# HKUST-Aerial-Robotics/FIESTA

Hardware: NVIDIA H100
Metric: esdf_voxel_updates_per_s (higher is better)
Workload: dtype int32+f64

## Files before the change

### fiesta_b200/csrc/fb_exact.cu

```cuda
#include <cub/cub.cuh>
#include <stdio.h>
#include <stdlib.h>
#include <algorithm>
#include <chrono>
#include "fb_common.cuh"
#include "fb_exact.h"

#define XNONE 0xffffffffu
#define XMB_NONE 0xffffffffffffffffull

__device__ __forceinline__ void x_coords(const FbGeom &g, uint32_t ii, int &x, int &y, int &z) {
  z = ii % (unsigned)g.pz; const unsigned xy = ii / (unsigned)g.pz; y = xy % (unsigned)g.gy; x = xy / (unsigned)g.gy;
}
__device__ __forceinline__ unsigned x_d2(int x, int y, int z, uint32_t c) {
  int ox, oy, oz; fb_unpack(c, ox, oy, oz); ox -= x; oy -= y; oz -= z;
  return (unsigned)(ox * ox + oy * oy + oz * oz);
}
__device__ __forceinline__ unsigned x_dist_of(int x, int y, int z, uint32_t c) { return c < 2u ? 0xffffffffu : x_d2(x, y, z, c); }

__global__ void k_x_flag_exist(const uint32_t *list, unsigned n, const double *occ, double l_occ, uint8_t *flags, int want) {
  const unsigned i = blockIdx.x * blockDim.x + threadIdx.x;
  if (i < n) flags[i] = ((occ[list[i]] > l_occ) ? 1 : 0) == want;
}
__global__ void k_x_apply_seed(FbGeom g, const uint32_t *E, unsigned n, uint32_t *cobs, unsigned long long *LS, unsigned long long t0) {
// ... 17 lines not shown
  const unsigned i = blockIdx.x * blockDim.x + threadIdx.x;
  if (i < n) scratch[sel[i]] = i;
}
__global__ void k_x_scan_deps(FbGeom g, const uint32_t *cobs, const uint32_t *occbits, const uint32_t *rank, const unsigned long long *LS,
                              unsigned long long *k1, unsigned long long *k2, uint32_t *dv, unsigned *ndep, unsigned cap, int shift) {
  for (long long v = (long long)blockIdx.x * blockDim.x + threadIdx.x; v < g.ptotal; v += (long long)gridDim.x * blockDim.x) {
    const uint32_t c = cobs[v] & FB_CODE_MASK;
    bool dep = false;
    unsigned r = 0;
    if (c >= 2u) {
      int ox, oy, oz; fb_unpack(c, ox, oy, oz);
      const long long oi = fb_ii(g, ox, oy, oz);
      if (!((__ldg(&occbits[oi >> 5]) >> (oi & 31)) & 1u)) { r = rank[oi]; dep = r != XNONE; }
    }
    const unsigned slot = fb_warp_append(ndep, dep);
    if (dep && slot < cap) {
      const unsigned long long inv = ~LS[v];
      if (shift) k1[slot] = ((unsigned long long)r << shift) | (inv & ((1ull << shift) - 1ull));
      else { k1[slot] = r; k2[slot] = inv; }
      dv[slot] = (uint32_t)v;
    }
  }
}
__global__ void k_x_unset(const uint32_t *list, unsigned n, uint32_t *scratch) {
  const unsigned i = blockIdx.x * blockDim.x + threadIdx.x;
  if (i < n) scratch[list[i]] = XNONE;
}
__global__ void k_x_iota(uint32_t *a, unsigned n) { const unsigned i = blockIdx.x * blockDim.x + threadIdx.x; if (i < n) a[i] = i; }
__global__ void k_x_gather64(const unsigned long long *src, const uint32_t *idx, unsigned n, unsigned long long *dst) {
  const unsigned i = blockIdx.x * blockDim.x + threadIdx.x; if (i < n) dst[i] = src[idx[i]];
}
__global__ void k_x_gather32(const uint32_t *src, const uint32_t *idx, unsigned n, uint32_t *dst) {
  const unsigned i = blockIdx.x * blockDim.x + threadIdx.x; if (i < n) dst[i] = src[idx[i]];
}
__global__ void k_x_set_ord(const uint32_t *deps, unsigned n, uint32_t *ord) {
  const unsigned i = blockIdx.x * blockDim.x + threadIdx.x;
  if (i < n) ord[deps[i]] = i;
}
__global__ void k_x_fill32(uint32_t *a, size_t n, uint32_t val) {
  for (size_t i = (size_t)blockIdx.x * blockDim.x + threadIdx.x; i < n; i += (size_t)gridDim.x * blockDim.x) a[i] = val;
}
__global__ void k_x_fill64(unsigned long long *a, size_t n, unsigned long long val) {
  for (size_t i = (size_t)blockIdx.x * blockDim.x + threadIdx.x; i < n; i += (size_t)gridDim.x * blockDim.x) a[i] = val;
}

static inline unsigned nblk(size_t n, unsigned t = 256) { return (unsigned)((n + t - 1) / t); }

static int x_select(FbExact *X, const uint32_t *in, const uint8_t *flags, uint32_t *out, unsigned n, unsigned *count, cudaStream_t s) {
  *count = 0;
  if (n == 0) return FIESTA_OK;
  size_t bytes = 0;
  CK(cub::DeviceSelect::Flagged(nullptr, bytes, in, flags, out, X->d_count.p, (int)n, s));
  CK(X->cub_tmp.grow(bytes, s));
  CK(cub::DeviceSelect::Flagged(X->cub_tmp.p, bytes, in, flags, out, X->d_count.p, (int)n, s));
  CK(cudaMemcpyAsync(X->h_count, X->d_count, 4, cudaMemcpyDeviceToHost, s));
  CK(cudaStreamSynchronize(s));
  *count = *X->h_count;
  return FIESTA_OK;
}
static int x_sort_pairs(FbExact *X, const unsigned long long *kin, unsigned long long *kout, const uint32_t *vin, uint32_t *vout, unsigned n, cudaStream_t s,
                        int key_bits = 64) {
  size_t bytes = 0;
  CK(cub::DeviceRadixSort::SortPairs(nullptr, bytes, kin, kout, vin, vout, (int)n, 0, key_bits, s));
  CK(X->cub_tmp.grow(bytes, s));
  CK(cub::DeviceRadixSort::SortPairs(X->cub_tmp.p, bytes, kin, kout, vin, vout, (int)n, 0, key_bits, s));
  return FIESTA_OK;
}
int fb_exact_init(FbExact *X, const FbGeom &g, int device, cudaStream_t s) {
  const size_t P = (size_t)g.ptotal;
  CK(fb_xrelax_init());
  X->relax_blocks = fb_xrelax_blocks(device);
  if (X->relax_blocks <= 0 || X->relax_blocks > FB_X_MAX_BLOCKS) { fb_set_error("exact mode init: k_x_relax does not fit on this device"); return FIESTA_ERR_CUDA; }
  CK(X->MB.alloc(P)); CK(X->LS.alloc(P)); CK(X->tkey.alloc(P));
  CK(X->touched.alloc(P));
  CK(X->SUM.alloc(P)); CK(X->SUMg.alloc(P)); CK(cudaMemsetAsync(X->SUMg, 0, P * 4, s));
  CK(X->emask.alloc(P));
  CK(X->wstamp.alloc(P)); CK(cudaMemsetAsync(X->wstamp, 0, P * 4, s));
  for (int k = 0; k < 3; ++k) { CK(X->W[k].alloc(P)); CK(X->F[k].alloc(P)); CK(cudaMemsetAsync(X->W[k], 0, P * 4, s)); }
  for (int k = 0; k < 2; ++k) CK(X->E[k].alloc(P));
  X->dense_min = 16384u;
  if (const char *e = getenv("FIESTA_X_DENSE")) { long v = atol(e); if (v >= 0 && v <= (1 << 24)) X->dense_min = (unsigned)v; }
  if (const char *e = getenv("FIESTA_X_ASYNC")) X->async = atol(e) != 0;
  if (const char *e = getenv("FIESTA_X_SMALL_ASYNC")) X->small_async = atol(e) != 0;
  X->small_max = FB_X_SMALL_DEFAULT;
  if (const char *e = getenv("FIESTA_X_SMALL")) { long v = atol(e); if (v >= 0 && v <= 65536) X->small_max = (unsigned)v; }
  CK(X->slotc.alloc(((size_t)X->small_max + 1) * 32));
  const size_t c0 = P / 8 > (1u << 20) ? P / 8 : (1u << 20);
  for (FbDevBuf<unsigned long long> *b : {&X->k1, &X->k2, &X->k1b, &X->k2b}) CK(b->grow(c0, s));
  for (FbDevBuf<uint32_t> *b : {&X->dv, &X->idx[0], &X->idx[1], &X->deps, &X->nc[0], &X->nc[1], &X->sel}) CK(b->grow(c0, s));
  CK(X->flags.grow(c0, s));
  CK(X->cub_tmp.grow(c0 * 16 + (64u << 20), s));
  CK(X->d_ctl.alloc(1)); CK(cudaMemsetAsync(X->d_ctl, 0, sizeof(FbXCtl), s));
  CK(X->h_ctl.alloc(1));
  CK(X->d_count.alloc(4)); CK(X->d_flag.alloc(4));
  CK(X->h_count.alloc(4));
  CK(cudaMemsetAsync(X->d_count, 0, 16, s)); CK(cudaMemsetAsync(X->d_flag, 0, 16, s));
  k_x_fill64<<<FB_SMS * 8, 256, 0, s>>>(X->MB, P, XMB_NONE);
  CK(cudaMemsetAsync(X->tkey, 0, P * 8, s));
  CK(cudaMemsetAsync(X->LS, 0, P * 8, s));
  X->tclock = 1; X->key_base = 0; X->key_epoch = 1; X->key_hi = 1ull << FB_KEY_BITS; X->gen_id = 0; X->wclock = 0; X->sclock = 0;
  CK(cudaGetLastError());
  return FIESTA_OK;
}

int fb_exact_queue_crossings(FbExact *X, const unsigned long long *ins_key, const uint32_t *ins_vox, const unsigned long long *del_key,
                             const uint32_t *del_vox, FbDevBuf<uint32_t> &ins, unsigned *n_ins, FbDevBuf<uint32_t> &del, unsigned *n_del,
                             cudaStream_t s, int *launches) {
  int r;
  CK(cudaMemcpyAsync(X->h_count, X->d_count, 8, cudaMemcpyDeviceToHost, s));
  CK(cudaStreamSynchronize(s));
  const unsigned ni = X->h_count[0], nd = X->h_count[1];
  CK(ins.grow((size_t)*n_ins + ni, s, *n_ins));
  CK(del.grow((size_t)*n_del + nd, s, *n_del));
  CK(X->k1b.grow(ni > nd ? ni : nd, s));
  if (ni) { if ((r = x_sort_pairs(X, ins_key, X->k1b, ins_vox, ins + *n_ins, ni, s, FB_KEY_BITS))) return r; *n_ins += ni; *launches += 1; }
  if (nd) { if ((r = x_sort_pairs(X, del_key, X->k1b, del_vox, del + *n_del, nd, s, FB_KEY_BITS))) return r; *n_del += nd; *launches += 1; }
  return FIESTA_OK;
}
int fb_exact_next_epoch(FbExact *X, const FbGeom &g, cudaStream_t s) {
  X->key_base = 0;
  if (++X->key_epoch >= (1u << (64 - FB_KEY_BITS))) {
    CK(cudaMemsetAsync(X->tkey, 0, (size_t)g.ptotal * 8, s));
    X->key_epoch = 1;
  }
  X->key_hi = (unsigned long long)X->key_epoch << FB_KEY_BITS;
  return FIESTA_OK;
}

int fb_exact_update_esdf(FbExact *X, const FbGeom &g, uint32_t *cobs, uint32_t *scratch, const double *occ, const uint32_t *occbits, double l_occ,
                         const uint32_t *ins, unsigned n_ins, const uint32_t *del, unsigned n_del, cudaStream_t s, FbExactStats *st, int *launches) {
  int r;
  const size_t P = (size_t)g.ptotal;
  memset(st, 0, sizeof(*st));
  CK(X->flags.grow((size_t)(n_ins > n_del ? n_ins : n_del) + 16, s));
  static const bool xdbg = getenv("FIESTA_DEBUG_X") != nullptr;
  auto now = [] { return std::chrono::steady_clock::now(); };
  auto ms = [](std::chrono::steady_clock::time_point a, std::chrono::steady_clock::time_point b) { return std::chrono::duration<double, std::milli>(b - a).count(); };
  const auto t_begin = now();
  unsigned nE = 0, ndep_run = 0;
  unsigned long long ls_deps = 0;
  bool scratch_ok = X->scratch_clean;
  if (n_ins) {
    k_x_flag_exist<<<nblk(n_ins), 256, 0, s>>>(ins, n_ins, occ, l_occ, X->flags, 1);
    if ((r = x_select(X, ins, X->flags, X->E[0], n_ins, &nE, s))) return r;
    if (nE) k_x_apply_seed<<<nblk(nE), 256, 0, s>>>(g, X->E[0], nE, cobs, X->LS, X->tclock);
    X->tclock += nE;
    *launches += 2;
  }
  if (n_del) {
    CK(X->sel.grow((size_t)n_del + 16, s));
    if (!X->scratch_clean) { k_x_fill32<<<FB_SMS * 8, 256, 0, s>>>(scratch, P, XNONE); *launches += 1; }
    scratch_ok = true;
    X->scratch_clean = false;
    k_x_del_minpos<<<nblk(n_del), 256, 0, s>>>(del, n_del, occ, l_occ, scratch);
    k_x_del_flag<<<nblk(n_del), 256, 0, s>>>(del, n_del, occ, l_occ, scratch, X->flags);
    unsigned nd = 0;
    if ((r = x_select(X, del, X->flags, X->sel, n_del, &nd, s))) return r;
    k_x_unset<<<nblk(n_del), 256, 0, s>>>(del, n_del, scratch);
    *launches += 3;
    if (nd) {
      k_x_del_rank<<<nblk(nd), 256, 0, s>>>(X->sel, nd, scratch);
      int rank_bits = 1; while ((1ull << rank_bits) < (unsigned long long)nd) ++rank_bits;
      int clock_bits = 1; while (clock_bits < 64 && (X->tclock >> clock_bits)) ++clock_bits;
      const bool two_sorts = getenv("FIESTA_X_TWO_SORTS") != nullptr;
      const int shift = (rank_bits + clock_bits <= 64 && !two_sorts) ? 64 - rank_bits : 0;
      unsigned ndep = 0;
      for (int attempt = 0; attempt < 2; ++attempt) {
        const size_t cap = std::min({X->dv.cap, X->k1.cap, X->k2.cap});
        CK(cudaMemsetAsync(X->d_count, 0, 4, s));
        k_x_scan_deps<<<FB_SMS * 16, 256, 0, s>>>(g, cobs, occbits, scratch, X->LS, X->k1, X->k2, X->dv, X->d_count, (unsigned)cap, shift);
        CK(cudaMemcpyAsync(X->h_count, X->d_count, 4, cudaMemcpyDeviceToHost, s));
        CK(cudaStreamSynchronize(s));
        ndep = *X->h_count;
        *launches += 1;
        if (ndep <= cap) break;
        CK(X->dv.grow(ndep, s));
        CK(X->k1.grow(ndep, s));
        CK(X->k2.grow(ndep, s));
      }
      st->dependants = ndep;
      k_x_unset<<<nblk(nd), 256, 0, s>>>(X->sel, nd, scratch);
      if (ndep) {
        CK(X->k1b.grow(ndep, s));
        CK(X->k2b.grow(ndep, s));
        CK(X->idx[0].grow(ndep, s));
        CK(X->idx[1].grow(ndep, s));
        CK(X->deps.grow(ndep, s));
        CK(X->nc[0].grow(ndep, s));
        CK(X->nc[1].grow(ndep, s));
        CK(X->flags.grow(ndep, s));
        if (shift) {
          if ((r = x_sort_pairs(X, X->k1, X->k1b, X->dv, X->deps, ndep, s))) return r;
          *launches += 1;
        } else {
          k_x_iota<<<nblk(ndep), 256, 0, s>>>(X->idx[0], ndep);
          if ((r = x_sort_pairs(X, X->k2, X->k2b, X->idx[0], X->idx[1], ndep, s))) return r;
          k_x_gather64<<<nblk(ndep), 256, 0, s>>>(X->k1, X->idx[1], ndep, X->k1b);
          if ((r = x_sort_pairs(X, X->k1b, X->k2b, X->idx[1], X->idx[0], ndep, s))) return r;
          k_x_gather32<<<nblk(ndep), 256, 0, s>>>(X->dv, X->idx[0], ndep, X->deps);
          *launches += 5;
        }
        k_x_set_ord<<<nblk(ndep), 256, 0, s>>>(X->deps, ndep, scratch);
        *launches += 1;
        ndep_run = ndep; ls_deps = X->tclock;
        X->tclock += ndep;
      }
    }
  }
  st->generations = 0;
  if (xdbg) { cudaStreamSynchronize(s); fprintf(stderr, "[x] seeds+deletes %.2f ms (dependants %u)\n", ms(t_begin, now()), st->dependants); }
  if (nE || ndep_run) {
    if (xdbg && !X->d_dbg) CK(X->d_dbg.alloc(FB_X_DBG_WORDS));
    if (xdbg) CK(cudaMemsetAsync(X->d_dbg, 0, FB_X_DBG_WORDS * 8, s));
    if (X->sclock > 0xf0000000u) { CK(cudaMemsetAsync(X->SUMg, 0, P * 4, s)); X->sclock = 0; }
    if (X->gen_id > 0xf0000000u) X->gen_id = 0;
    if (X->wclock > 0xf0000000u) { CK(cudaMemsetAsync(X->wstamp, 0, P * 4, s)); X->wclock = 0; }
    FbXCtl *h = X->h_ctl;
    memset(h, 0, sizeof(*h));
    h->gen_id = X->gen_id; h->wclock = X->wclock; h->tclock = X->tclock; h->sclock = X->sclock; h->nE0 = nE;
    CK(cudaMemcpyAsync(X->d_ctl, h, sizeof(FbXCtl), cudaMemcpyHostToDevice, s));
    CK(fb_xrelax_launch(X, g, cobs, X->deps, ndep_run, scratch, X->nc[0], X->nc[1], occbits, ls_deps, xdbg ? X->d_dbg.p : nullptr, s));
    if (ndep_run) k_x_unset<<<nblk(ndep_run), 256, 0, s>>>(X->deps, ndep_run, scratch);
    CK(cudaMemcpyAsync(h, X->d_ctl, sizeof(FbXCtl), cudaMemcpyDeviceToHost, s));
    CK(cudaStreamSynchronize(s));
    *launches += ndep_run ? 2 : 1;
    if (h->err) {
      if (h->err == 3u) {
        for (int k = 0; k < 3; ++k) CK(cudaMemsetAsync(X->W[k], 0, P * 4, s));
        CK(cudaMemsetAsync(X->wstamp, 0, P * 4, s));
        X->wclock = 0;
      }
      fb_set_error(h->err == 1u ? "exact mode: generation with more than 2^27 entries"
                   : h->err == 3u ? "exact mode: a wait of the asynchronous work queue exceeded its bound" : "exact mode: behaviour fixpoint did not converge");
      return FIESTA_ERR_CUDA;
    }
    X->gen_id = h->gen_id; X->wclock = h->wclock; X->tclock = h->tclock; X->sclock = h->sclock;
    st->generations = h->generations; st->reseed_rounds = h->reseed_rounds; st->eval_rounds = h->rounds; st->dense_rounds = h->dense_rounds;
    st->voxels_changed = h->voxels_changed; st->expansions = h->expansions;
    if (xdbg) {
      static unsigned long long hd[FB_X_DBG_WORDS];
      static double cyc_per_us = 0;
      if (cyc_per_us == 0) { int dev = 0, khz = 0; CK(cudaGetDevice(&dev)); CK(cudaDeviceGetAttribute(&khz, cudaDevAttrClockRate, dev)); cyc_per_us = khz / 1000.0; }
      CK(cudaMemcpy(hd, X->d_dbg, sizeof(hd), cudaMemcpyDeviceToHost));
      static const char *cat[FB_XDBG_NCAT] = {"S", "round1", "rounds", "dense", "commit", "apply", "s.round1", "s.rounds", "s.commit", "s.apply", "top",
                                              "empty-barrier", "reseed.classify", "reseed.assemble", "", "", "async", "", "refresh", "s.async",
                                              "reseed.closure", "reseed.choose", "reseed.resolve", ""};
      fprintf(stderr, "[x] reseed rounds %u; phases (us, count):", st->reseed_rounds);
      for (int c = 0; c < FB_XDBG_NCAT; ++c)
        if (*cat[c]) fprintf(stderr, " %s %.0f/%llu", cat[c], hd[FB_XDBG_PHASE + 2 * c] / cyc_per_us, hd[FB_XDBG_PHASE + 2 * c + 1]);
      fprintf(stderr, "\n");
      fprintf(stderr, "[x] round work (summed longest CTA work time us / summed list length):");
      for (int c : {1, 2, 3, 6, 7}) fprintf(stderr, " %s %.0f/%llu", cat[c], hd[FB_XDBG_WORK + 2 * c] / cyc_per_us, hd[FB_XDBG_WORK + 2 * c + 1]);
      fprintf(stderr, "\n");
      for (int h = 0; h < 2; ++h) {
        fprintf(stderr, "[x] list-length histogram %s (log2 bucket=rounds):", h ? "s.rounds" : "rounds");
        for (int b = 0; b < 32; ++b) if (hd[FB_XDBG_NWH + 32 * h + b]) fprintf(stderr, " %d=%llu", b, hd[FB_XDBG_NWH + 32 * h + b]);
        fprintf(stderr, "\n");
      }
      fprintf(stderr, "[x] async: evaluations %llu dirty %llu pushes %llu spin %.0f us\n", hd[FB_XDBG_Q + 0], hd[FB_XDBG_Q + 1], hd[FB_XDBG_Q + 2],
              hd[FB_XDBG_Q + 3] / cyc_per_us);
      for (int gq = 0; gq < 2; ++gq) { fprintf(stderr, "[x] gen %d work lists:", gq); for (int r = 0; r < 512 && hd[FB_XDBG_ROUNDS + gq * 512 + r]; ++r) fprintf(stderr, " %llu", hd[FB_XDBG_ROUNDS + gq * 512 + r]); fprintf(stderr, "\n"); }
      fprintf(stderr, "[x] work-list entries: evaluated %llu refreshed %llu\n", hd[FB_XDBG_PHASE + 2 * 14], hd[FB_XDBG_PHASE + 2 * 14 + 1]);
      fprintf(stderr, "[x] reseed: dependants %u final after classify %llu closure rounds %llu list entries %llu resolve passes %llu\n", st->dependants,
              hd[FB_XDBG_PHASE + 2 * 15], hd[FB_XDBG_PHASE + 2 * 20 + 1], hd[FB_XDBG_PHASE + 2 * 15 + 1], hd[FB_XDBG_PHASE + 2 * 22 + 1]);
      fprintf(stderr, "[x] gens %u rounds %u dense %u deps %u nE0 %u |", st->generations, st->eval_rounds, st->dense_rounds, st->dependants, nE);
      for (unsigned q = 0; q < st->generations && q < FB_XDBG_GENS; ++q) fprintf(stderr, " %llu/%llu/%.1fus", hd[3 * q], hd[3 * q + 1], hd[3 * q + 2] / cyc_per_us);
      fprintf(stderr, "\n");
    }
  }
  X->scratch_clean = scratch_ok;
  return FIESTA_OK;
}
```

### fiesta_b200/csrc/fb_exact.h

```cpp
#pragma once
#include "fb_common.cuh"

#define FB_X_MAX_BLOCKS 256
#define FB_X_SMALL_DEFAULT 32768u
#define FB_XDBG_GENS 1024
#define FB_XDBG_NCAT 24
#define FB_XDBG_NQ 8
#define FB_XDBG_PHASE (3 * FB_XDBG_GENS)
#define FB_XDBG_ROUNDS (FB_XDBG_PHASE + 2 * FB_XDBG_NCAT)
#define FB_XDBG_WMAX (FB_XDBG_ROUNDS + 2 * 512)
#define FB_XDBG_WORK (FB_XDBG_WMAX + 4096)
#define FB_XDBG_NWH (FB_XDBG_WORK + 2 * FB_XDBG_NCAT)
#define FB_XDBG_Q (FB_XDBG_NWH + 2 * 32)
#define FB_X_DBG_WORDS (FB_XDBG_Q + FB_XDBG_NQ)

struct FbExactStats {
  unsigned long long expansions;
  unsigned long long voxels_changed;
  unsigned generations, eval_rounds, dense_rounds, dependants;
  unsigned reseed_rounds;
};

struct FbXCtl {
  unsigned bar, err;
  unsigned sclock;
  unsigned rbar;
  unsigned nE0;
  unsigned nW[3], nF[3];
  unsigned gen_id, wclock;
  unsigned generations, rounds, dense_rounds, reseed_rounds;
  unsigned long long tclock, expansions, voxels_changed;
  unsigned partial[FB_X_MAX_BLOCKS];
  alignas(128) unsigned long long qtail;
  alignas(128) unsigned qhead;
  alignas(128) unsigned qdone;
};

struct FbExact {
  FbDevBuf<unsigned long long> MB;
  FbDevBuf<unsigned long long> LS;
  FbDevBuf<unsigned long long> tkey;
  FbDevBuf<uint32_t> touched;
  unsigned long long tclock = 0;
  unsigned long long key_base = 0;
  unsigned long long key_hi = 0;
  unsigned key_epoch = 0;
  FbDevBuf<unsigned> d_count, d_flag;
  FbHostBuf<unsigned> h_count;
  bool scratch_clean = false;
  FbDevBuf<uint4> SUM;
  FbDevBuf<uint32_t> SUMg;
  unsigned gen_id = 0, wclock = 0, sclock = 0;
  FbDevBuf<uint32_t> emask;
  FbDevBuf<uint32_t> W[3], F[3];
  FbDevBuf<uint32_t> wstamp;
  FbDevBuf<uint32_t> slotc;
  unsigned dense_min = 0;
  unsigned small_max = 0;
  bool async = true;
  bool small_async = false;
  FbDevBuf<FbXCtl> d_ctl;
  FbHostBuf<FbXCtl> h_ctl;
  FbDevBuf<unsigned long long> d_dbg;
  int relax_blocks = 0;
  FbDevBuf<uint32_t> E[2], sel;
  FbDevBuf<unsigned long long> k1, k2, k1b, k2b;
  FbDevBuf<uint32_t> dv, idx[2], deps, nc[2];
  FbDevBuf<uint8_t> flags;
  FbDevBuf<char> cub_tmp;
};

int fb_exact_init(FbExact *X, const FbGeom &g, int device, cudaStream_t s);
int fb_exact_queue_crossings(FbExact *X, const unsigned long long *ins_key, const uint32_t *ins_vox, const unsigned long long *del_key,
                             const uint32_t *del_vox, FbDevBuf<uint32_t> &ins, unsigned *n_ins, FbDevBuf<uint32_t> &del, unsigned *n_del,
                             cudaStream_t s, int *launches);
int fb_exact_next_epoch(FbExact *X, const FbGeom &g, cudaStream_t s);
int fb_exact_update_esdf(FbExact *X, const FbGeom &g, uint32_t *cobs, uint32_t *scratch, const double *occ, const uint32_t *occbits, double l_occ,
                         const uint32_t *ins, unsigned n_ins, const uint32_t *del, unsigned n_del, cudaStream_t s, FbExactStats *st, int *launches);
cudaError_t fb_xrelax_init();
int fb_xrelax_blocks(int device);
cudaError_t fb_xrelax_launch(FbExact *X, const FbGeom &g, uint32_t *cobs, const uint32_t *deps, unsigned ndep, uint32_t *ord, uint32_t *nc, uint32_t *M,
                             const uint32_t *occbits, unsigned long long ls_deps, unsigned long long *dbg, cudaStream_t s);
```

### fiesta_b200/csrc/fb_xrelax.cu

```cuda
#include <stdio.h>
#include "fb_common.cuh"
#include "fb_exact.h"
#include "fb_divmagic.h"

#define XT 1024
#define XW (XT / 32)
#define XNONE 0xffffffffu
#define X_DEAD 0ull
#define X_PULL 1ull
#define X_PUSH 2ull
#define XMB_NONE 0xffffffffffffffffull
#define X_NOFF 129
#define X_MAX_ROUNDS 4000000u
#define XGB 8
#define XDBG_PHASE FB_XDBG_PHASE
#define XDBG_ROUNDS FB_XDBG_ROUNDS
#define XDBG_WMAX FB_XDBG_WMAX

static __constant__ int x_dirs[24][3] = {
    {-1, 0, 0}, {1, 0, 0}, {0, -1, 0}, {0, 1, 0}, {0, 0, -1}, {0, 0, 1},
    {-1, -1, 0}, {1, 1, 0}, {0, -1, -1}, {0, 1, 1}, {-1, 0, -1}, {1, 0, 1},
    {-1, 1, 0}, {1, -1, 0}, {0, -1, 1}, {0, 1, -1}, {1, 0, -1}, {-1, 0, 1},
    {-2, 0, 0}, {2, 0, 0}, {0, -2, 0}, {0, 2, 0}, {0, 0, -2}, {0, 0, 2}};
static __constant__ int x_off_c[X_NOFF];
// ... 67 lines not shown
      for (int j = 0; j < XGB; ++j) w[j] = x_writer_word(g, MB, v, x, y, z, XGB * h + j, inr);
    }
#pragma unroll
    for (int j = 0; j < XGB; ++j) {
      const unsigned long long ww = w[j];
      if (ww == XMB_NONE || x_mb_kind(ww) != X_PUSH) continue;
      const unsigned ts = x_mb_idx(ww) * 32u + (unsigned)(XGB * h + j);
      const uint32_t c = x_mb_code(ww);
      const unsigned d = x_d2(x, y, z, c);
      if (d < d0) {
        if (WANT_FIRST && ts < first) first = ts;
        if (ts < T && (d < s.d || (d == s.d && ts < s.ts))) { s.d = d; s.c = c; s.ts = ts; }
      }
    }
  }
  if (wown != XMB_NONE && x_mb_kind(wown) == X_PULL) {
    const unsigned ts = x_mb_idx(wown) * 32u + 24u;
    const uint32_t c = x_mb_code(wown);
    const unsigned d = x_d2(x, y, z, c);
    if (d < d0) {
      if (WANT_FIRST && ts < first) first = ts;
      if (ts < T && (d < s.d || (d == s.d && ts < s.ts))) { s.d = d; s.c = c; s.ts = ts; }
    }
  }
  return s;
}
__device__ __forceinline__ void x_summarize(const FbGeom &g, const uint32_t *cobs, const unsigned long long *MB, uint4 *SUM, int x, int y, int z) {
  unsigned first; uint32_t snap;
  const XState f = x_gather<true>(g, cobs, MB, x, y, z, XNONE, first, snap);
  SUM[x_vi(g, x, y, z)] = make_uint4(first, f.ts, f.c, snap);
}
template <bool USE_SUM>
__device__ __forceinline__ XState x_state(const FbGeom &g, const uint32_t *cobs, const unsigned long long *MB, const uint4 *SUM, int x, int y, int z,
                                          unsigned T, uint32_t &snap) {
  unsigned first;
  if (USE_SUM) {
    const uint4 u = __ldcg(&SUM[x_vi(g, x, y, z)]);
    snap = u.w;
    XState s;
    if (u.x == XNONE || T <= u.x) { s.c = u.w; s.d = x_dist_of(x, y, z, s.c); s.ts = XNONE; return s; }
    if (T > u.y) { s.c = u.z; s.d = x_dist_of(x, y, z, s.c); s.ts = u.y; return s; }
  }
  return x_gather<false>(g, cobs, MB, x, y, z, T, first, snap);
}

__device__ __forceinline__ unsigned x_ld_acquire(const unsigned *p) {
  unsigned v;
  asm volatile("ld.acquire.gpu.global.u32 %0, [%1];" : "=r"(v) : "l"(p) : "memory");
  return v;
}
__device__ __forceinline__ void x_gsync(unsigned *bar, unsigned &target) {
  __syncthreads();
  if (threadIdx.x == 0) {
    target += gridDim.x;
    asm volatile("red.release.gpu.global.add.u32 [%0], %1;" ::"l"(bar), "r"(1u) : "memory");
    while (x_ld_acquire(bar) < target) { }
  }
  __syncthreads();
}

struct XArgs {
  FbGeom g;
  uint32_t *cobs;
  unsigned long long *MB, *LS;
  uint4 *SUM;
  uint32_t *SUMg;
  uint32_t *E[2];
  uint32_t *emask;
  uint32_t *W[3], *F[3];
  uint32_t *wstamp;
  uint32_t *slotc;
  FbXCtl *ctl;
  unsigned small_max, dense_min;
  const uint32_t *deps; unsigned ndep;
  uint32_t *ord;
  uint32_t *nc;
  uint32_t *M;
  const uint32_t *occbits;
  unsigned long long ls_deps;
  unsigned long long *dbg;
  unsigned div_pz_m, div_pz_s, div_gy_m, div_gy_s;
  unsigned async_on;
  unsigned small_async_on;
};
__device__ __forceinline__ unsigned x_div(unsigned n, unsigned m, unsigned s) { return m ? (__umulhi(n, m) >> s) : n; }
__device__ __forceinline__ void x_coords(const XArgs &a, uint32_t ii, int &x, int &y, int &z) {
  const unsigned xy = x_div(ii, a.div_pz_m, a.div_pz_s);
  z = (int)(ii - xy * (unsigned)a.g.pz);
  const unsigned xx = x_div(xy, a.div_gy_m, a.div_gy_s);
  y = (int)(xy - xx * (unsigned)a.g.gy);
  x = (int)xx;
}

__device__ __forceinline__ void x_unpack_off(int o, int &dx, int &dy, int &dz) { dx = (o & 15) - 4; dy = ((o >> 4) & 15) - 4; dz = ((o >> 8) & 15) - 4; }

__device__ __forceinline__ void x_claim_summaries(const XArgs &a, const XShared &sh, unsigned lane, int x, int y, int z, unsigned sclock) {
  if (lane >= 25u) return;
  int dx, dy, dz; x_unpack_off(sh.dir[lane], dx, dy, dz);
  const int nx = x + dx, ny = y + dy, nz = z + dz;
  if (!x_in_grid(a.g, nx, ny, nz) || !(lane == 24u || x_in_range(a.g, nx, ny, nz))) return;
  const unsigned n = x_vi(a.g, nx, ny, nz);
  if (__ldcg(&a.SUMg[n]) != sclock && atomicExch(&a.SUMg[n], sclock) != sclock) x_summarize(a.g, a.cobs, a.MB, a.SUM, nx, ny, nz);
}

__device__ __forceinline__ void x_refresh_summaries(const XArgs &a, const XShared &sh, unsigned lane, unsigned i, uint32_t p, int x, int y, int z) {
  unsigned long long w = 0;
  if (lane == 0) w = __ldcg(&a.MB[p]);
  w = __shfl_sync(0xffffffffu, w, 0);
  if (lane >= 25u) return;
  int dx, dy, dz; x_unpack_off(sh.dir[lane], dx, dy, dz);
  const int nx = x + dx, ny = y + dy, nz = z + dz;
  if (!x_in_grid(a.g, nx, ny, nz) || !(lane == 24u || x_in_range(a.g, nx, ny, nz))) return;
  const uint4 u = __ldcg(&a.SUM[x_vi(a.g, nx, ny, nz)]);
  if (u.w == FB_UNKNOWN) return;
  const unsigned ts = i * 32u + lane;
  bool redo = u.x == ts || u.y == ts;
  if (!redo) {
    const unsigned long long kind = x_mb_kind(w);
    const uint32_t c = x_mb_code(w);
    if (((kind == X_PUSH && lane < 24u) || (kind == X_PULL && lane == 24u)) && c >= 2u) {
      const unsigned d = x_d2(nx, ny, nz, c);
      if (u.y == XNONE) redo = true;
      else { const unsigned bd = x_d2(nx, ny, nz, u.z); redo = ts < u.x || d < bd || (d == bd && ts < u.y); }
    }
  }
  if (redo) x_summarize(a.g, a.cobs, a.MB, a.SUM, nx, ny, nz);
}

__device__ __forceinline__ void x_list_affected(const XArgs &a, const XShared &sh, unsigned lane, unsigned i, int x, int y, int z, unsigned nof,
                                                unsigned wclock, unsigned out) {
  const FbGeom &g = a.g;
  unsigned long long w[5];
#pragma unroll
  for (int t = 0; t < 5; ++t) {
    const unsigned o = lane + 32u * (unsigned)t;
    w[t] = XMB_NONE;
    if (o < nof) {
      int dx, dy, dz; x_unpack_off(sh.off[o], dx, dy, dz);
      const int nx = x + dx, ny = y + dy, nz = z + dz;
      if (x_in_grid(g, nx, ny, nz)) w[t] = __ldcg(&a.MB[x_vi(g, nx, ny, nz)]);
    }
  }
  unsigned j[5], st[5];
#pragma unroll
  for (int t = 0; t < 5; ++t) {
    j[t] = w[t] != XMB_NONE ? x_mb_idx(w[t]) : 0u;
    st[t] = (w[t] != XMB_NONE && j[t] > i) ? __ldcg(&a.wstamp[j[t]]) : wclock;
  }
  unsigned pm = 0;
#pragma unroll
  for (int t = 0; t < 5; ++t)
    if (st[t] != wclock && atomicExch(&a.wstamp[j[t]], wclock) != wclock) pm |= 1u << t;
  const unsigned cnt = (unsigned)__popc(pm);
  unsigned incl = cnt;
#pragma unroll
  for (int o = 1; o < 32; o <<= 1) { const unsigned v = __shfl_up_sync(0xffffffffu, incl, o); if ((int)lane >= o) incl += v; }
  const unsigned total = __shfl_sync(0xffffffffu, incl, 31);
  if (total == 0u) return;
  unsigned base = 0;
  if (lane == 0) base = atomicAdd(&a.ctl->nW[out], total);
  base = __shfl_sync(0xffffffffu, base, 0) + incl - cnt;
#pragma unroll
  for (int t = 0; t < 5; ++t) if ((pm >> t) & 1u) a.W[out][base++] = j[t];
}

template <bool USE_SUM>
// ... 311 lines not shown
    __threadfence();
    while (om) {
      const unsigned i = s0 + (unsigned)(__ffs(om) - 1) * nwk;
      om &= om - 1u;
      x_q_run<false, DBG>(a, sh, stg, lane, E, nE, ring, gen, A, 0u, i, true);
    }
  }
  if (lane == 0) x_q_count(a, sh, 0ull - (1ull << 32));
  unsigned h = XNONE;
  for (;;) {
    unsigned i = 0;
    if (lane == 0) i = x_q_take<DBG>(a, sh, ring, nE, h);
    i = __shfl_sync(0xffffffffu, i, 0);
    if (i == XNONE) break;
    x_q_run<false, DBG>(a, sh, stg, lane, E, nE, ring, gen, A, 0u, i, false);
    if (lane == 0) x_q_count(a, sh, 0ull - (1ull << 32));
  }
}

extern __shared__ __align__(16) unsigned char x_dyn_smem[];

#define X_STATIC 0x20000000u
#define X_VALID 0x40000000u
#define X_PAR 0x80000000u
#define X_LAP(cat) do { if (DBG && gtid == 0) { const long long t_now = clock64(); a.dbg[XDBG_PHASE + 2 * (cat)] += (unsigned long long)(t_now - t_ph); a.dbg[XDBG_PHASE + 2 * (cat) + 1] += 1ull; t_ph = t_now; } } while (0)

template <int K0>
__device__ __forceinline__ void x_dep_nb(const XArgs &a, int x, int y, int z, unsigned want, unsigned (&nv)[8], unsigned (&o)[8]) {
#pragma unroll
  for (int t = 0; t < 8; ++t) {
    const int nx = x + x_dc(K0 + t, 0), ny = y + x_dc(K0 + t, 1), nz = z + x_dc(K0 + t, 2);
    nv[t] = ((want >> (K0 + t)) & 1u) && x_in_grid(a.g, nx, ny, nz) && x_in_range(a.g, nx, ny, nz) ? x_vi(a.g, nx, ny, nz) : XNONE;
    o[t] = nv[t] != XNONE ? __ldcg(&a.ord[nv[t]]) : XNONE;
  }
}
template <int K0>
__device__ __forceinline__ unsigned x_first_valid(const XArgs &a, int x, int y, int z, unsigned mask, unsigned &par) {
  unsigned nv[8], o[8], m[8];
  x_dep_nb<K0>(a, x, y, z, mask, nv, o);
#pragma unroll
  for (int t = 0; t < 8; ++t) m[t] = o[t] != XNONE ? __ldcg(&a.M[o[t]]) : 0u;
#pragma unroll
  for (int t = 0; t < 8; ++t) if (m[t] & X_VALID) { par = o[t]; return (unsigned)(K0 + t); }
  return 24u;
}
template <int K0>
__device__ __forceinline__ void x_classify(const XArgs &a, unsigned i, int x, int y, int z, unsigned &mask, uint32_t &sc, bool &done) {
  unsigned nv[8], o[8];
  uint32_t c[8];
  x_dep_nb<K0>(a, x, y, z, 0xffffffu, nv, o);
#pragma unroll
  for (int t = 0; t < 8; ++t) c[t] = (nv[t] != XNONE && o[t] == XNONE) ? __ldcg(&a.cobs[nv[t]]) & FB_CODE_MASK : 0u;
  unsigned e[8];
#pragma unroll
  for (int t = 0; t < 8; ++t) {
    e[t] = 0u;
    if (c[t] >= 2u) { int ox, oy, oz; fb_unpack(c[t], ox, oy, oz); const unsigned oi = x_vi(a.g, ox, oy, oz); e[t] = (__ldg(&a.occbits[oi >> 5]) >> (oi & 31)) & 1u; }
  }
#pragma unroll
  for (int t = 0; t < 8; ++t) {
    if (done || nv[t] == XNONE) continue;
    if (o[t] != XNONE) { if (o[t] < i) mask |= 1u << (K0 + t); }
    else if (e[t]) { sc = c[t]; done = true; }
  }
}
template <int K0>
__device__ __forceinline__ void x_mark_later(const XArgs &a, bool act, unsigned o, int x, int y, int z, unsigned out) {
  unsigned j[8], m[8];
#pragma unroll
  for (int t = 0; t < 8; ++t) {
    const int nx = x + x_dc(K0 + t, 0), ny = y + x_dc(K0 + t, 1), nz = z + x_dc(K0 + t, 2);
    j[t] = act && x_in_grid(a.g, nx, ny, nz) ? __ldcg(&a.ord[x_vi(a.g, nx, ny, nz)]) : XNONE;
  }
#pragma unroll
  for (int t = 0; t < 8; ++t) m[t] = (j[t] != XNONE && j[t] > o) ? __ldcg(&a.M[j[t]]) : X_VALID;
#pragma unroll
  for (int t = 0; t < 8; ++t) {
    const bool push = !(m[t] & (X_STATIC | X_VALID)) && !(atomicOr(&a.M[j[t]], X_VALID) & X_VALID);
    const unsigned slot = fb_warp_append(&a.ctl->nW[out], push);
    if (push) a.W[out][slot] = j[t];
  }
}

template <bool DBG>
__global__ void __launch_bounds__(XT, 1) k_x_reseed(const XArgs a) {
  __shared__ XShared sh;
  FbXCtl *ctl = a.ctl;
  const unsigned tid = threadIdx.x, lane = tid & 31u, wid = tid >> 5, G = gridDim.x, b = blockIdx.x;
  const unsigned gtid = b * XT + tid, gthreads = G * XT;
  unsigned bar_target = 0;
  long long t_ph = DBG ? clock64() : 0;
  for (unsigned i0 = 0; i0 < a.ndep; i0 += gthreads) {
    const unsigned i = i0 + gtid;
    unsigned mask = 0;
    uint32_t sc = FB_INF;
    bool done = true;
    if (i < a.ndep) {
      int x, y, z; x_coords(a, __ldcg(&a.deps[i]), x, y, z);
      done = false;
      x_classify<0>(a, i, x, y, z, mask, sc, done);
      if (!done) x_classify<8>(a, i, x, y, z, mask, sc, done);
      if (!done) x_classify<16>(a, i, x, y, z, mask, sc, done);
      a.nc[i] = sc;
      a.M[i] = mask | (done ? X_STATIC | X_VALID : 0u);
    }
    const bool pull = !done && mask;
    const unsigned slot = fb_warp_append(&ctl->nW[1], pull);
    if (pull) a.W[1][slot] = i;
    if (DBG) { const unsigned f = __popc(__ballot_sync(0xffffffffu, i < a.ndep && !mask)); if ((threadIdx.x & 31u) == 0 && f) atomicAdd(&a.dbg[XDBG_PHASE + 2 * 15], (unsigned long long)f); }
  }
  x_gsync(&ctl->rbar, bar_target);
  X_LAP(12);
  unsigned r = 1, rounds = 0;
  for (;; ++r) {
    const unsigned in = r % 3u, out = (r + 1u) % 3u, zz = (r + 2u) % 3u;
    const unsigned nw = __ldcg(&ctl->nW[in]);
    if (gtid == 0) ctl->nW[zz] = 0;
    if (nw == 0u) break;
    ++rounds;
    if (DBG && gtid == 0) a.dbg[XDBG_PHASE + 2 * 15 + 1] += nw;
    for (unsigned q0 = 0; q0 < nw; q0 += gthreads) {
      const unsigned q = q0 + gtid;
      const bool act = q < nw;
      const unsigned i = act ? __ldcg(&a.W[in][q]) : 0u;
      int x = 0, y = 0, z = 0;
      if (act) x_coords(a, __ldcg(&a.deps[i]), x, y, z);
      if (r == 1u) {
        unsigned k = 24u, par;
        if (act) {
          const unsigned mask = __ldcg(&a.M[i]);
          k = x_first_valid<0>(a, x, y, z, mask, par);
          if (k == 24u) k = x_first_valid<8>(a, x, y, z, mask, par);
          if (k == 24u) k = x_first_valid<16>(a, x, y, z, mask, par);
          if (k != 24u) a.M[i] = mask | X_VALID;
        }
        const unsigned slot = fb_warp_append(&ctl->nW[out], k != 24u);
        if (k != 24u) a.W[out][slot] = i;
      } else {
        const bool push = act && x_in_range(a.g, x, y, z);
        x_mark_later<0>(a, push, i, x, y, z, out);
        x_mark_later<8>(a, push, i, x, y, z, out);
        x_mark_later<16>(a, push, i, x, y, z, out);
      }
    }
    x_gsync(&ctl->rbar, bar_target);
    X_LAP(20);
  }
  {
    const unsigned out = (r + 1u) % 3u;
    for (unsigned i0 = 0; i0 < a.ndep; i0 += gthreads) {
      const unsigned i = i0 + gtid;
      const unsigned m = i < a.ndep ? __ldcg(&a.M[i]) : 0u;
      unsigned k = 24u, par = 0;
      if ((m & X_VALID) && (m & 0xffffffu)) {
        int x, y, z; x_coords(a, __ldcg(&a.deps[i]), x, y, z);
        k = x_first_valid<0>(a, x, y, z, m, par);
        if (k == 24u) k = x_first_valid<8>(a, x, y, z, m, par);
        if (k == 24u) k = x_first_valid<16>(a, x, y, z, m, par);
        if (k != 24u) a.nc[i] = X_PAR | par;
      }
      const unsigned slot = fb_warp_append(&ctl->nW[out], k != 24u);
      if (k != 24u) a.W[out][slot] = i;
    }
    x_gsync(&ctl->rbar, bar_target);
    X_LAP(21);
  }
  unsigned passes = 0;
  for (++r;; ++r) {
    const unsigned in = r % 3u, out = (r + 1u) % 3u, zz = (r + 2u) % 3u;
    const unsigned nw = __ldcg(&ctl->nW[in]);
    if (gtid == 0) ctl->nW[zz] = 0;
    if (nw == 0u) break;
    ++passes;
    for (unsigned q0 = 0; q0 < nw; q0 += gthreads) {
      const unsigned q = q0 + gtid;
      bool again = false;
      unsigned i = 0;
      if (q < nw) {
        i = __ldcg(&a.W[in][q]);
        const uint32_t c = __ldcg(&a.nc[__ldcg(&a.nc[i]) & ~X_PAR]);
        a.nc[i] = c;
        again = (c & X_PAR) != 0u;
      }
      const unsigned slot = fb_warp_append(&ctl->nW[out], again);
      if (again) a.W[out][slot] = i;
    }
    x_gsync(&ctl->rbar, bar_target);
    X_LAP(22);
  }
  const unsigned per = (a.ndep + G - 1u) / G;
  const unsigned lo = min(a.ndep, b * per), hi = min(a.ndep, lo + per);
  unsigned mine = 0;
  for (unsigned i = lo + tid; i < hi; i += XT) mine += __ldcg(&a.nc[i]) >= 2u ? 1u : 0u;
  unsigned tot;
  x_block_scan(sh, mine, lane, wid, tot);
  if (tid == 0) ctl->partial[b] = tot;
  const unsigned nE = __ldcg(&ctl->nE0);
  x_gsync(&ctl->rbar, bar_target);
  if (wid == 0) {
    unsigned before = 0, all = 0;
    for (unsigned k = lane; k < G; k += 32u) { const unsigned c = __ldcg(&ctl->partial[k]); all += c; if (k < b) before += c; }
#pragma unroll
    for (int o = 16; o > 0; o >>= 1) { before += __shfl_xor_sync(0xffffffffu, before, o); all += __shfl_xor_sync(0xffffffffu, all, o); }
    if (lane == 0) { sh.base = before; sh.total = all; }
  }
  __syncthreads();
  unsigned run = nE + sh.base;
  for (unsigned i0 = lo; i0 < hi; i0 += XT) {
    const unsigned i = i0 + tid;
    uint32_t c = FB_INF, v = 0;
    if (i < hi) {
      c = __ldcg(&a.nc[i]); v = __ldcg(&a.deps[i]);
      a.cobs[v] = c;
      a.LS[v] = a.ls_deps + i;
    }
    unsigned ctot;
    const unsigned pos = x_block_scan(sh, (i < hi && c >= 2u) ? 1u : 0u, lane, wid, ctot);
    if (i < hi && c >= 2u) a.E[0][run + pos] = v;
    run += ctot;
  }
  if (gtid == 0) {
    ctl->nE0 = nE + sh.total;
    ctl->reseed_rounds = rounds + passes;
    ctl->nW[0] = ctl->nW[1] = ctl->nW[2] = 0;
  }
  X_LAP(13);
}

template <bool DBG>
__global__ void __launch_bounds__(XT, 1) k_x_relax(const XArgs a) {
  __shared__ XShared sh;
  const FbGeom &g = a.g;
  FbXCtl *ctl = a.ctl;
  const unsigned tid = threadIdx.x, lane = tid & 31u, wid = tid >> 5;
  const unsigned G = gridDim.x, b = blockIdx.x;
  const unsigned gtid = b * XT + tid, gthreads = G * XT;
  const unsigned gwarp = gtid >> 5, gwarps = gthreads >> 5;
  for (unsigned k = tid; k < X_NOFF; k += XT) sh.off[k] = x_off_c[k];
  if (tid < 32) sh.self[tid] = 0;
  if (tid == 0) sh.qdone = 0u;
  if (gtid == 0) a.ctl->qtail = (unsigned long long)gwarps << 32;
  if (tid < 32) sh.dir[tid] = tid < 24 ? ((x_dirs[tid][0] + 4) | ((x_dirs[tid][1] + 4) << 4) | ((x_dirs[tid][2] + 4) << 8)) : (4 | (4 << 4) | (4 << 8));
  __syncthreads();
  for (unsigned q = tid; q < 25u * 24u + 25u; q += XT) {
    const unsigned t = q < 600u ? q / 24u : q - 600u, k = q < 600u ? q % 24u : 24u;
    int tx, ty, tz, kx = 0, ky = 0, kz = 0; x_unpack_off(sh.dir[t], tx, ty, tz);
    if (k < 24u) x_unpack_off(sh.dir[k], kx, ky, kz);
    const int code = (tx - kx + 4) | ((ty - ky + 4) << 4) | ((tz - kz + 4) << 8);
    unsigned found = 0;
    for (unsigned o = 0; o < X_NOFF; ++o) if (sh.off[o] == code) found = o;
    if (q < 600u) sh.slot[q] = (unsigned char)found; else sh.self[t] = (unsigned char)found;
  }
  __syncthreads();
  XNb &stg = reinterpret_cast<XNb *>(x_dyn_smem)[wid];

  unsigned nE = ctl->nE0, bar_target = 0;
  int cur = 0;
  unsigned gen = ctl->gen_id, wclock = ctl->wclock;
  unsigned long long tclock = ctl->tclock;
  unsigned generations = 0, rounds_total = 0, dense_total = 0;
  unsigned long long changed_total = 0;
  if (DBG) {
    const long long t0 = clock64();
    for (int q = 0; q < 32; ++q) x_gsync(&ctl->bar, bar_target);
    if (gtid == 0) a.dbg[XDBG_PHASE + 2 * 11] = (unsigned long long)(clock64() - t0) / 32ull;
  }
  long long t_ph = DBG ? clock64() : 0;
  bool big = nE > a.small_max;

  ++gen;
  unsigned sclock = ctl->sclock;
  for (unsigned i = gtid; i < nE; i += gthreads) {
    const uint32_t v = __ldcg(&a.E[0][i]);
    a.MB[v] = x_mb(gen, i, X_PUSH, __ldcg(&a.cobs[v]) & FB_CODE_MASK);
  }
  x_gsync(&ctl->bar, bar_target);

  while (nE) {
    const long long t_gen = DBG ? clock64() : 0;
    X_LAP(10);
    ++generations;
    const uint32_t *E = a.E[cur];
    unsigned rounds = 0;
    bool aborted = false;
    if (big) {
      ++sclock;
      for (unsigned i = gwarp; i < nE; i += gwarps) { int x, y, z; x_coords(a, __ldcg(&E[i]), x, y, z); x_claim_summaries(a, sh, lane, x, y, z, sclock); }
      x_gsync(&ctl->bar, bar_target);
      X_LAP(0);
    }
    for (unsigned r = 1;; ++r) {
      const unsigned in = r % 3u, out = (r + 1u) % 3u, zz = (r + 2u) % 3u;
      const unsigned nw = r == 1u ? nE : __ldcg(&ctl->nW[in]);
      const unsigned nf = (big && r > 1u) ? __ldcg(&ctl->nF[in]) : 0u;
      if (gtid == 0) { ctl->nW[zz] = 0; ctl->nF[zz] = 0; }
      if (r > 1u && nw == 0u && nf == 0u) break;
      if (r > X_MAX_ROUNDS) { if (gtid == 0) ctl->err = 2u; break; }
      if (DBG && gtid == 0) { a.dbg[XDBG_PHASE + 2 * 14] += nw; a.dbg[XDBG_PHASE + 2 * 14 + 1] += nf; }
      if (a.async_on && (big ? r > 1u && nw <= a.dense_min : r == 1u && a.small_async_on)) {
        ++rounds; wclock += 3u;
        const unsigned A = wclock - 1u;
        if (big) x_async<DBG>(a, sh, stg, lane, gwarp, gwarps, E, nE, a.W[in], nw, a.W[out], gen, A, out);
        else x_async_small<DBG>(a, sh, stg, lane, gwarp, gwarps, E, nE, a.W[out], gen, A);
        x_gsync(&ctl->bar, bar_target);
        X_LAP(big ? 16 : 19);
        if (tid == 0) sh.qdone = 0u;
        if (gtid == 0) { ctl->qtail = (unsigned long long)gwarps << 32; ctl->qhead = 0u; ctl->qdone = 0u; }
        if (__ldcg(&ctl->err)) { aborted = true; break; }
        if (!big) break;
        const unsigned nfa = __ldcg(&ctl->nF[out]);
        if (nfa > (unsigned)g.ptotal) {
          ++sclock;
          for (unsigned i = gwarp; i < nE; i += gwarps) { int x, y, z; x_coords(a, __ldcg(&E[i]), x, y, z); x_claim_summaries(a, sh, lane, x, y, z, sclock); }
        } else {
          for (unsigned q = gwarp; q < nf + nfa; q += gwarps) {
            const unsigned i = q < nf ? __ldcg(&a.F[in][q]) : __ldcg(&a.F[out][q - nf]);
            const uint32_t p = __ldcg(&E[i]);
            int x, y, z; x_coords(a, p, x, y, z);
            x_refresh_summaries(a, sh, lane, i, p, x, y, z);
          }
// ... 135 lines not shown
      if (m) {
        const uint32_t p = __ldcg(&E[i]);
        int x, y, z; x_coords(a, p, x, y, z);
        uint32_t me = m;
        while (me) {
          const int k = __ffs(me) - 1; me &= me - 1u;
          int dx, dy, dz; x_unpack_off(sh.dir[k], dx, dy, dz);
          const uint32_t v = (uint32_t)x_vi(g, x + dx, y + dy, z + dz);
          const unsigned ts = i * 32u + (unsigned)k;
          const uint32_t code = big ? __ldcg(&a.SUM[v]).z : __ldcg(&a.slotc[ts]);
          a.cobs[v] = code;
          a.LS[v] = tclock + ts;
          En[r] = v;
          a.MB[v] = x_mb(gen + 1u, r, X_PUSH, code);
          ++r;
        }
      }
      run += ctot;
    }
    if (DBG && gtid == 0 && generations <= FB_XDBG_GENS) { a.dbg[3 * (generations - 1u)] = nE; a.dbg[3 * (generations - 1u) + 1] = rounds; a.dbg[3 * (generations - 1u) + 2] = (unsigned long long)(clock64() - t_gen); }
    tclock += (unsigned long long)nE * 32ull + 1ull;
    changed_total += n2;
    if (n2 >= (1u << 27)) { if (gtid == 0) ctl->err = 1u; break; }
    const bool was_big = big;
    nE = n2; cur ^= 1; big = big2; ++gen;
    x_gsync(&ctl->bar, bar_target);
    X_LAP(was_big ? 5 : 9);
  }
  if (gtid == 0) {
    ctl->gen_id = gen; ctl->wclock = wclock; ctl->tclock = tclock; ctl->sclock = sclock;
    ctl->generations = generations; ctl->rounds = rounds_total; ctl->dense_rounds = dense_total; ctl->voxels_changed = changed_total;
  }
}

static bool g_off_ready = false;
cudaError_t fb_xrelax_init() {
  if (g_off_ready) return cudaSuccess;
  static const int D[24][3] = {
      {-1, 0, 0}, {1, 0, 0}, {0, -1, 0}, {0, 1, 0}, {0, 0, -1}, {0, 0, 1},
      {-1, -1, 0}, {1, 1, 0}, {0, -1, -1}, {0, 1, 1}, {-1, 0, -1}, {1, 0, 1},
      {-1, 1, 0}, {1, -1, 0}, {0, -1, 1}, {0, 1, -1}, {1, 0, -1}, {-1, 0, 1},
      {-2, 0, 0}, {2, 0, 0}, {0, -2, 0}, {0, 2, 0}, {0, 0, -2}, {0, 0, 2}};
  int off[1024], n = 0;
  for (int p = -1; p < 24; ++p)
    for (int q = -1; q < 24; ++q) {
      int o[3];
      for (int k = 0; k < 3; ++k) o[k] = (p < 0 ? 0 : D[p][k]) + (q < 0 ? 0 : D[q][k]);
      const int code = (o[0] + 4) | ((o[1] + 4) << 4) | ((o[2] + 4) << 8);
      bool dup = false;
      for (int j = 0; j < n; ++j) dup = dup || off[j] == code;
      if (!dup) off[n++] = code;
    }
  if (n != X_NOFF) return cudaErrorUnknown;
  cudaError_t e = cudaMemcpyToSymbol(x_off_c, off, sizeof(int) * X_NOFF);
  if (e == cudaSuccess) g_off_ready = true;
  return e;
}

int fb_xrelax_blocks(int device) {
  int per_sm = 0, sms = 0;
  for (const void *k : {(const void *)k_x_relax<false>, (const void *)k_x_relax<true>})
    if (cudaOccupancyMaxActiveBlocksPerMultiprocessor(&per_sm, k, XT, sizeof(XNb) * XW) != cudaSuccess || per_sm < 1) return -1;
  for (const void *k : {(const void *)k_x_reseed<false>, (const void *)k_x_reseed<true>})
    if (cudaOccupancyMaxActiveBlocksPerMultiprocessor(&per_sm, k, XT, 0) != cudaSuccess || per_sm < 1) return -1;
  if (cudaDeviceGetAttribute(&sms, cudaDevAttrMultiProcessorCount, device) != cudaSuccess) return -1;
  return sms;
}

cudaError_t fb_xrelax_launch(FbExact *X, const FbGeom &g, uint32_t *cobs, const uint32_t *deps, unsigned ndep, uint32_t *ord, uint32_t *nc, uint32_t *M,
                             const uint32_t *occbits, unsigned long long ls_deps, unsigned long long *dbg, cudaStream_t s) {
  XArgs a;
  a.deps = deps; a.ndep = ndep; a.ord = ord; a.nc = nc; a.M = M; a.occbits = occbits; a.ls_deps = ls_deps;
  fb_div_make((unsigned)g.pz, a.div_pz_m, a.div_pz_s);
  fb_div_make((unsigned)g.gy, a.div_gy_m, a.div_gy_s);
  a.g = g;
  if (a.g.max_vec[0] < a.g.min_vec[0] || a.g.max_vec[1] < a.g.min_vec[1] || a.g.max_vec[2] < a.g.min_vec[2])
    for (int k = 0; k < 3; ++k) a.g.min_vec[k] = a.g.max_vec[k] = 0x3fffffff;
  a.cobs = cobs; a.MB = X->MB; a.LS = X->LS; a.SUM = X->SUM; a.SUMg = X->SUMg;
  a.E[0] = X->E[0]; a.E[1] = X->E[1]; a.emask = X->emask;
  for (int k = 0; k < 3; ++k) { a.W[k] = X->W[k]; a.F[k] = X->F[k]; }
  a.wstamp = X->wstamp; a.slotc = X->slotc; a.ctl = X->d_ctl; a.small_max = X->small_max; a.dense_min = X->dense_min; a.dbg = dbg;
  a.async_on = X->async ? 1u : 0u;
  a.small_async_on = X->small_async ? 1u : 0u;
  void *args[] = {(void *)&a};
  if (ndep) {
    const cudaError_t e = cudaLaunchCooperativeKernel(dbg ? (void *)k_x_reseed<true> : (void *)k_x_reseed<false>, dim3(X->relax_blocks), dim3(XT), args, 0, s);
    if (e != cudaSuccess) return e;
  }
  return cudaLaunchCooperativeKernel(dbg ? (void *)k_x_relax<true> : (void *)k_x_relax<false>, dim3(X->relax_blocks), dim3(XT), args, sizeof(XNb) * XW, s);
}
```

Before: 140.3 million.

## Replace round-synchronous reseed closure with an asynchronous device-wide work queue

The reseed closure no longer advances level by level with a grid-wide barrier per round. After the first round, warps pull entries from a global ring buffer, and new dependants are appended with atomic tail counters and done/abort flags. This is meant to remove the per-round grid synchronisation cost on long dependency chains. In exchange it adds spin-wait polling, a timeout abort path, and extra atomics. It is enabled by default and can be switched off with FIESTA_X_RESEED_ASYNC.

```diff
diff --git a/fiesta_b200/csrc/fb_exact.cu b/fiesta_b200/csrc/fb_exact.cu
--- a/fiesta_b200/csrc/fb_exact.cu
+++ b/fiesta_b200/csrc/fb_exact.cu
@@ -123,6 +123,7 @@
   if (const char *e = getenv("FIESTA_X_DENSE")) { long v = atol(e); if (v >= 0 && v <= (1 << 24)) X->dense_min = (unsigned)v; }
   if (const char *e = getenv("FIESTA_X_ASYNC")) X->async = atol(e) != 0;
   if (const char *e = getenv("FIESTA_X_SMALL_ASYNC")) X->small_async = atol(e) != 0;
+  if (const char *e = getenv("FIESTA_X_RESEED_ASYNC")) X->reseed_async = atol(e) != 0;
   X->small_max = FB_X_SMALL_DEFAULT;
   if (const char *e = getenv("FIESTA_X_SMALL")) { long v = atol(e); if (v >= 0 && v <= 65536) X->small_max = (unsigned)v; }
   CK(X->slotc.alloc(((size_t)X->small_max + 1) * 32));
@@ -285,7 +286,7 @@
       CK(cudaMemcpy(hd, X->d_dbg, sizeof(hd), cudaMemcpyDeviceToHost));
       static const char *cat[FB_XDBG_NCAT] = {"S", "round1", "rounds", "dense", "commit", "apply", "s.round1", "s.rounds", "s.commit", "s.apply", "top",
                                               "empty-barrier", "reseed.classify", "reseed.assemble", "", "", "async", "", "refresh", "s.async",
-                                              "reseed.closure", "reseed.choose", "reseed.resolve", ""};
+                                              "reseed.closure", "reseed.choose", "reseed.resolve", "reseed.queue"};
       fprintf(stderr, "[x] reseed rounds %u; phases (us, count):", st->reseed_rounds);
       for (int c = 0; c < FB_XDBG_NCAT; ++c)
         if (*cat[c]) fprintf(stderr, " %s %.0f/%llu", cat[c], hd[FB_XDBG_PHASE + 2 * c] / cyc_per_us, hd[FB_XDBG_PHASE + 2 * c + 1]);
diff --git a/fiesta_b200/csrc/fb_exact.h b/fiesta_b200/csrc/fb_exact.h
--- a/fiesta_b200/csrc/fb_exact.h
+++ b/fiesta_b200/csrc/fb_exact.h
@@ -34,6 +34,9 @@
   alignas(128) unsigned long long qtail;
   alignas(128) unsigned qhead;
   alignas(128) unsigned qdone;
+  alignas(128) unsigned long long rtail;
+  alignas(128) unsigned rhead;
+  alignas(128) unsigned rdone;
 };
 
 struct FbExact {
@@ -59,6 +62,7 @@
   unsigned small_max = 0;
   bool async = true;
   bool small_async = false;
+  bool reseed_async = true;
   FbDevBuf<FbXCtl> d_ctl;
   FbHostBuf<FbXCtl> h_ctl;
   FbDevBuf<unsigned long long> d_dbg;
diff --git a/fiesta_b200/csrc/fb_xrelax.cu b/fiesta_b200/csrc/fb_xrelax.cu
--- a/fiesta_b200/csrc/fb_xrelax.cu
+++ b/fiesta_b200/csrc/fb_xrelax.cu
@@ -173,6 +173,7 @@
   unsigned div_pz_m, div_pz_s, div_gy_m, div_gy_s;
   unsigned async_on;
   unsigned small_async_on;
+  unsigned reseed_async_on;
 };
 __device__ __forceinline__ unsigned x_div(unsigned n, unsigned m, unsigned s) { return m ? (__umulhi(n, m) >> s) : n; }
 __device__ __forceinline__ void x_coords(const XArgs &a, uint32_t ii, int &x, int &y, int &z) {
@@ -650,6 +651,96 @@
   }
 }
 
+__device__ __forceinline__ void x_st_relaxed(unsigned *p, unsigned v) { asm volatile("st.relaxed.gpu.global.u32 [%0], %1;" ::"l"(p), "r"(v) : "memory"); }
+__device__ __forceinline__ void x_rq_abort(const XArgs &a) {
+  atomicCAS(&a.ctl->err, 0u, 3u);
+  atomicExch(&a.ctl->rdone, 1u);
+}
+__device__ __forceinline__ unsigned x_rq_count(const XArgs &a, XShared &sh, unsigned long long delta) {
+  const unsigned long long old = atomicAdd(&a.ctl->rtail, delta);
+  if ((unsigned)((old + delta) >> 32) == 0u) { atomicExch(&a.ctl->rdone, 1u); sh.qdone = 1u; }
+  return (unsigned)old;
+}
+template <bool DBG>
+__device__ __forceinline__ void x_mark_later_q(const XArgs &a, XShared &sh, unsigned lane, bool act, unsigned o, int x, int y, int z, uint32_t *ring,
+                                               uint32_t *depth, unsigned d, unsigned fin) {
+  unsigned j[24];
+#pragma unroll
+  for (int t = 0; t < 24; ++t) {
+    const int nx = x + x_dc(t, 0), ny = y + x_dc(t, 1), nz = z + x_dc(t, 2);
+    j[t] = act && x_in_grid(a.g, nx, ny, nz) ? __ldcg(&a.ord[x_vi(a.g, nx, ny, nz)]) : XNONE;
+  }
+  unsigned pm = 0;
+#pragma unroll
+  for (int t = 0; t < 24; ++t)
+    if (j[t] != XNONE && j[t] > o && !(atomicOr(&a.M[j[t]], X_VALID) & X_VALID)) pm |= 1u << t;
+  const unsigned cnt = (unsigned)__popc(pm);
+  unsigned incl = cnt;
+#pragma unroll
+  for (int s = 1; s < 32; s <<= 1) { const unsigned v = __shfl_up_sync(0xffffffffu, incl, s); if ((int)lane >= s) incl += v; }
+  const unsigned total = __shfl_sync(0xffffffffu, incl, 31);
+  unsigned base = 0;
+  if (lane == 0) base = x_rq_count(a, sh, (unsigned long long)total * 0x100000001ull - ((unsigned long long)fin << 32));
+  base = __shfl_sync(0xffffffffu, base, 0) + incl - cnt;
+  if (DBG && pm) {
+#pragma unroll
+    for (int t = 0; t < 24; ++t) if ((pm >> t) & 1u) depth[j[t]] = d;
+    __threadfence();
+  }
+#pragma unroll
+  for (int t = 0; t < 24; ++t) if ((pm >> t) & 1u) x_st_relaxed(&ring[base++], j[t] | X_Q_FULL);
+}
+template <bool DBG>
+__device__ void x_reseed_queue(const XArgs &a, XShared &sh, unsigned lane, uint32_t *ring, uint32_t *depth) {
+  const volatile unsigned *done = &sh.qdone;
+  for (;;) {
+    unsigned base = 0;
+    if (lane == 0) base = atomicAdd(&a.ctl->rhead, 32u);
+    base = __shfl_sync(0xffffffffu, base, 0);
+    if (base >= a.ndep) return;
+    const unsigned idx = base + lane;
+    unsigned pend = __ballot_sync(0xffffffffu, idx < a.ndep);
+    unsigned long long t0 = 0;
+    unsigned ns = 32;
+    for (unsigned it = 0; pend;) {
+      const unsigned v = (pend >> lane) & 1u ? x_ld_relaxed(&ring[idx]) : 0u;
+      const bool got = (v & X_Q_FULL) != 0u;
+      const unsigned gm = __ballot_sync(0xffffffffu, got);
+      if (gm) {
+        pend &= ~gm;
+        const unsigned o = v & ~X_Q_FULL;
+        int x = 0, y = 0, z = 0;
+        if (got) { ring[idx] = 0u; x_coords(a, __ldcg(&a.deps[o]), x, y, z); }
+        unsigned d = 0;
+        if (DBG) {
+          if (got) { __threadfence(); d = __ldcg(&depth[o]) + 1u; }
+          const unsigned dm = __reduce_max_sync(0xffffffffu, d);
+          if (lane == 0) atomicMax(&a.dbg[FB_XDBG_Q + 4], (unsigned long long)(dm - 1u));
+        }
+        const bool push = got && x_in_range(a.g, x, y, z);
+        x_mark_later_q<DBG>(a, sh, lane, push, o, x, y, z, ring, depth, d, (unsigned)__popc(gm));
+        t0 = 0; ns = 32;
+        continue;
+      }
+      unsigned stop = 0;
+      if (lane == 0) {
+        stop = *done;
+        if (!stop && (++it & 15u) == 0u) {
+          if (x_ld_acquire(&a.ctl->rdone)) { sh.qdone = 1u; stop = 1u; }
+          else {
+            const unsigned long long t = x_globaltimer();
+            if (t0 == 0) t0 = t;
+            else if (t - t0 > X_Q_WAIT_NS) { x_rq_abort(a); sh.qdone = 1u; stop = 1u; }
+          }
+        }
+      }
+      if (__shfl_sync(0xffffffffu, stop, 0)) return;
+      __nanosleep(ns);
+      ns = ns < 256u ? 2u * ns : 256u;
+    }
+  }
+}
+
 template <bool DBG>
 __global__ void __launch_bounds__(XT, 1) k_x_reseed(const XArgs a) {
   __shared__ XShared sh;
@@ -658,6 +749,7 @@
   const unsigned gtid = b * XT + tid, gthreads = G * XT;
   unsigned bar_target = 0;
   long long t_ph = DBG ? clock64() : 0;
+  if (tid == 0) sh.qdone = 0u;
   for (unsigned i0 = 0; i0 < a.ndep; i0 += gthreads) {
     const unsigned i = i0 + gtid;
     unsigned mask = 0;
@@ -702,8 +794,16 @@
           if (k == 24u) k = x_first_valid<16>(a, x, y, z, mask, par);
           if (k != 24u) a.M[i] = mask | X_VALID;
         }
-        const unsigned slot = fb_warp_append(&ctl->nW[out], k != 24u);
-        if (k != 24u) a.W[out][slot] = i;
+        if (a.reseed_async_on) {
+          const unsigned pm = __ballot_sync(0xffffffffu, k != 24u);
+          unsigned base = 0;
+          if (lane == 0 && pm) base = (unsigned)atomicAdd(&ctl->rtail, (unsigned long long)__popc(pm) * 0x100000001ull);
+          base = __shfl_sync(0xffffffffu, base, 0) + (unsigned)__popc(pm & ((1u << lane) - 1u));
+          if (k != 24u) { a.W[2][base] = i | X_Q_FULL; if (DBG) a.W[0][i] = 1u; }
+        } else {
+          const unsigned slot = fb_warp_append(&ctl->nW[out], k != 24u);
+          if (k != 24u) a.W[out][slot] = i;
+        }
       } else {
         const bool push = act && x_in_range(a.g, x, y, z);
         x_mark_later<0>(a, push, i, x, y, z, out);
@@ -713,6 +813,21 @@
     }
     x_gsync(&ctl->rbar, bar_target);
     X_LAP(20);
+    if (r == 1u && a.reseed_async_on) {
+      const unsigned n1 = (unsigned)__ldcg(&ctl->rtail);
+      if (n1 == 0u) continue;
+      x_reseed_queue<DBG>(a, sh, lane, a.W[2], a.W[0]);
+      x_gsync(&ctl->rbar, bar_target);
+      X_LAP(23);
+      if (__ldcg(&ctl->err)) return;
+      if (DBG) {
+        const unsigned chain = (unsigned)__ldcg(&a.dbg[FB_XDBG_Q + 4]);
+        rounds += chain;
+        if (gtid == 0) { a.dbg[XDBG_PHASE + 2 * 20 + 1] += chain; a.dbg[XDBG_PHASE + 2 * 15 + 1] += (unsigned)__ldcg(&ctl->rtail); }
+      } else {
+        ++rounds;
+      }
+    }
   }
   {
     const unsigned out = (r + 1u) % 3u;
@@ -804,6 +919,7 @@
   const unsigned G = gridDim.x, b = blockIdx.x;
   const unsigned gtid = b * XT + tid, gthreads = G * XT;
   const unsigned gwarp = gtid >> 5, gwarps = gthreads >> 5;
+  if (__ldcg(&ctl->err)) return;
   for (unsigned k = tid; k < X_NOFF; k += XT) sh.off[k] = x_off_c[k];
   if (tid < 32) sh.self[tid] = 0;
   if (tid == 0) sh.qdone = 0u;
@@ -1105,6 +1221,7 @@
   a.wstamp = X->wstamp; a.slotc = X->slotc; a.ctl = X->d_ctl; a.small_max = X->small_max; a.dense_min = X->dense_min; a.dbg = dbg;
   a.async_on = X->async ? 1u : 0u;
   a.small_async_on = X->small_async ? 1u : 0u;
+  a.reseed_async_on = X->reseed_async ? 1u : 0u;
   void *args[] = {(void *)&a};
   if (ndep) {
     const cudaError_t e = cudaLaunchCooperativeKernel(dbg ? (void *)k_x_reseed<true> : (void *)k_x_reseed<false>, dim3(X->relax_blocks), dim3(XT), args, 0, s);
```

After: 143.6 million, median of 6. +2.4%, better.
